# IvanAnishchuk/eth-consensus-specs

Hardware: AMD Instinct MI355X
Metric: BLS sig verifications/sec (FastAggregateVerify, 1/8 GPU) + % int VALU peak (higher is better)
Workload: dtype u32 (381-bit Montgomery Fp, radix-2^29 digits); 1 GPU; C2 sync-committee FastAggregateVerify: 10000 aggregates x 512 pubkeys per GPU; config=c2, global_batch=10000, registry=1048576, parallelism=dp1 (sharded, RCCL all-gather of 576-B Fp12 partials)

## Files before the change

__graft_entry__.py:

```python
import os
import subprocess
import sys

ROOT = os.path.dirname(os.path.abspath(__file__))
PKG = os.path.join(ROOT, "eth-consensus-specs_amd")


def _paths():
    for p in (ROOT, PKG):
        if p not in sys.path:
            sys.path.insert(0, p)


def build() -> None:
    subprocess.check_call(["make", "-C", PKG, "-j8"], timeout=3000)
    subprocess.check_call(["make", "-j2", "-C", os.path.join(ROOT, "tests", "hostcheck")], timeout=3000)
    subprocess.check_call(["make", "-C", os.path.join(ROOT, "tests", "hostcheck_endo")], timeout=3000)
    subprocess.check_call(["make", "-C", os.path.join(ROOT, "tests", "hostcheck_mlines")], timeout=3000)
    subprocess.check_call(["make", "-C", os.path.join(ROOT, "tests", "hostcheck_segsum")], timeout=3000)
    subprocess.check_call(["make", "-C", os.path.join(ROOT, "tests", "hostcheck_g2segsum")], timeout=3000)
    subprocess.check_call(["make", "-C", os.path.join(ROOT, "tests", "hostcheck_g1dot")], timeout=3000)
    subprocess.check_call(["make", "-C", os.path.join(ROOT, "tests", "hostcheck_bits")], timeout=3000)
    subprocess.check_call(["make", "-C", os.path.join(ROOT, "oracle")], timeout=3000)
    subprocess.check_call(["make", "-j3", "-C", os.path.join(ROOT, "tests", "sanitize")], timeout=3000)
    _paths()
    import bls_mi355x
    from bls_mi355x import _native
    _native.load_library()


def smoke() -> None:
    _paths()
    import hashlib

    from bls_mi355x import batch
    from bls_mi355x import bls as shim
    from oracle import bls_oracle as O

    n = 64
    sks = b"".join((i + 1).to_bytes(32, "big") for i in range(n))
    pks = batch.sk_to_pk_batch(sks)
    assert pks[:48] == O.SkToPk(1)
    batch.Registry().load(pks)
    committees = [list(range(0, 16)), list(range(16, 48)), list(range(48, 64))]
    msgs = [hashlib.sha256(bytes([j])).digest() for j in range(3)]
    agg = [sum(k + 1 for k in c) % O.R for c in committees]
    sigs = bytearray(batch.sign_batch(b"".join(a.to_bytes(32, "big") for a in agg), b"".join(msgs)))
    sigs[96:192] = sigs[192:288]
    idx = [k for c in committees for k in c]
    offs = batch.offsets_from_lengths([len(c) for c in committees])
    out = batch.fast_aggregate_verify_batch(idx, offs, b"".join(msgs), bytes(sigs))
    expect = [O.FastAggregateVerify([pks[48 * k: 48 * k + 48] for k in c], m, bytes(sigs[96 * j: 96 * j + 96]))
              for j, (c, m) in enumerate(zip(committees, msgs))]
    assert list(out) == expect == [True, False, True], (list(out), expect)
    pk, m = O.SkToPk(7), b"\x12" * 32
    assert shim.Verify(pk, m, O.Sign(7, m)) is True
    print("smoke ok:", list(out))


if __name__ == "__main__":
    build()
    if len(sys.argv) > 1 and sys.argv[1] == "smoke":
        smoke()
```

eth-consensus-specs_amd/csrc/bls_fq.h:

```cpp
#pragma once
#include "bls_fp.h"
#include "bls_fq_constants.h"

#ifdef BLS_FQ_CHECK
#include <assert.h>
#endif

namespace bls {

constexpr uint32_t Q29_MASK = 0x1fffffffu;

#ifdef BLS_FQ_CHECK
inline double fq_check_top(const Fq& a) {
  double v = 0;
  for (int i = 0; i < 14; ++i) v += (double)a.d[i] * __builtin_ldexp(1.0, 29 * i - 377);
  return v;
}
inline void fq_check_mul(const Fq& x, const Fq& y) {
  assert(fq_check_top(x) * fq_check_top(y) < 13.0 * __builtin_ldexp(1.0, 29));
}
#define FQ_CHECK_MUL(x, y) fq_check_mul(x, y)
inline void fq_check_dot2(const Fq& x, const Fq& y, const Fq& u, const Fq& v) {
  assert(fq_check_top(x) * fq_check_top(y) + fq_check_top(u) * fq_check_top(v) < 13.0 * __builtin_ldexp(1.0, 29));
}
#define FQ_CHECK_DOT2(x, y, u, v) fq_check_dot2(x, y, u, v)
#define FQ_CHECK_COL(acc128) assert((acc128) < ((unsigned __int128)1 << 64))
#define FQ_CHECK_SUB(b, K)                                        \
  do {                                                            \
    for (int i_ = 0; i_ < 14; ++i_) assert((b).d[i_] <= (K)[i_]); \
  } while (0)
#else
#define FQ_CHECK_MUL(x, y) ((void)0)
#define FQ_CHECK_DOT2(x, y, u, v) ((void)0)
#define FQ_CHECK_COL(acc128) ((void)0)
#define FQ_CHECK_SUB(b, K) ((void)0)
#endif

BLS_HD Fq fq_zero() {
  Fq r;
#pragma unroll
  for (int i = 0; i < 14; i++) r.d[i] = 0;
  return r;
}

BLS_HD Fq fq_select(bool c, const Fq& a, const Fq& b) {
  Fq r;
#pragma unroll
  for (int i = 0; i < 14; i++) r.d[i] = c ? a.d[i] : b.d[i];
  return r;
}

BLS_HD Fq fq_add(const Fq& a, const Fq& b) {
  Fq r;
#pragma unroll
  for (int i = 0; i < 14; i++) r.d[i] = a.d[i] + b.d[i];
  return r;
}

BLS_HD Fq fq_sub(const Fq& a, const Fq& b) {
  FQ_CHECK_SUB(b, Q29_K1);
  Fq r;
#pragma unroll
  for (int i = 0; i < 14; i++) r.d[i] = a.d[i] + (Q29_K1[i] - b.d[i]);
  return r;
}

BLS_HD Fq fq_sub2(const Fq& a, const Fq& b) {
  FQ_CHECK_SUB(b, Q29_K2);
  Fq r;
#pragma unroll
  for (int i = 0; i < 14; i++) r.d[i] = a.d[i] + (Q29_K2[i] - b.d[i]);
  return r;
}

BLS_HD Fq fq_norm(const Fq& a) {
  Fq r;
  r.d[0] = a.d[0] & Q29_MASK;
#pragma unroll
  for (int i = 1; i < 13; i++) r.d[i] = (a.d[i] & Q29_MASK) + (a.d[i - 1] >> 29);
  r.d[13] = a.d[13] + (a.d[12] >> 29);
  return r;
}

BLS_HD Fq fq_mul_small(const Fq& a, uint32_t k) {
  uint64_t t[14];
#pragma unroll
  for (int i = 0; i < 14; i++) t[i] = (uint64_t)a.d[i] * k;
  Fq r;
  r.d[0] = (uint32_t)t[0] & Q29_MASK;
#pragma unroll
  for (int i = 1; i < 13; i++) r.d[i] = ((uint32_t)t[i] & Q29_MASK) + (uint32_t)(t[i - 1] >> 29);
  r.d[13] = (uint32_t)t[13] + (uint32_t)(t[12] >> 29);
  return r;
}

BLS_HD Fq fq_mul(const Fq& x, const Fq& y) {
  FQ_CHECK_MUL(x, y);
  uint32_t m[14];
  Fq r;
  uint64_t acc = 0;
#pragma unroll
  for (int k = 0; k < 27; k++) {
#ifdef BLS_FQ_CHECK
    unsigned __int128 chk = acc;
#endif
#pragma unroll
    for (int i = 0; i < 14; i++) {
      const int j = k - i;
      if (j >= 0 && j < 14) {
        acc += (uint64_t)x.d[i] * y.d[j];
#ifdef BLS_FQ_CHECK
        chk += (unsigned __int128)x.d[i] * y.d[j];
#endif
      }
    }
#pragma unroll
    for (int i = 0; i < 14; i++) {
      const int j = k - i;
      if (j >= 1 && j < 14 && i < k) {
        acc += (uint64_t)m[i] * P29[j];
#ifdef BLS_FQ_CHECK
        chk += (unsigned __int128)m[i] * P29[j];
#endif
      }
    }
    if (k < 14) {
      m[k] = ((uint32_t)acc * P29_NINV) & Q29_MASK;
      acc += (uint64_t)m[k] * P29[0];
#ifdef BLS_FQ_CHECK
      chk += (unsigned __int128)m[k] * P29[0];
#endif
    } else {
      r.d[k - 14] = (uint32_t)acc & Q29_MASK;
    }
    FQ_CHECK_COL(chk);
    acc >>= 29;
  }
  r.d[13] = (uint32_t)acc;
  return r;
}

BLS_HD Fq fq_mul_dot2(const Fq& x, const Fq& y, const Fq& u, const Fq& v) {
  FQ_CHECK_DOT2(x, y, u, v);
  uint32_t m[14];
  Fq r;
  uint64_t acc = 0;
#pragma unroll
  for (int k = 0; k < 27; k++) {
#ifdef BLS_FQ_CHECK
    unsigned __int128 chk = acc;
#endif
#pragma unroll
    for (int i = 0; i < 14; i++) {
      const int j = k - i;
      if (j >= 0 && j < 14) {
        acc += (uint64_t)x.d[i] * y.d[j];
        acc += (uint64_t)u.d[i] * v.d[j];
#ifdef BLS_FQ_CHECK
        chk += (unsigned __int128)x.d[i] * y.d[j] + (unsigned __int128)u.d[i] * v.d[j];
#endif
      }
    }
#pragma unroll
    for (int i = 0; i < 14; i++) {
      const int j = k - i;
      if (j >= 1 && j < 14 && i < k) {
        acc += (uint64_t)m[i] * P29[j];
#ifdef BLS_FQ_CHECK
        chk += (unsigned __int128)m[i] * P29[j];
#endif
      }
    }
    if (k < 14) {
      m[k] = ((uint32_t)acc * P29_NINV) & Q29_MASK;
      acc += (uint64_t)m[k] * P29[0];
#ifdef BLS_FQ_CHECK
      chk += (unsigned __int128)m[k] * P29[0];
#endif
    } else {
      r.d[k - 14] = (uint32_t)acc & Q29_MASK;
    }
    FQ_CHECK_COL(chk);
    acc >>= 29;
  }
  r.d[13] = (uint32_t)acc;
  return r;
}

BLS_HD Fq fq_sqr(const Fq& x) {
  FQ_CHECK_MUL(x, x);
  uint32_t m[14];
  Fq r;
  uint64_t acc = 0;
#pragma unroll
  for (int k = 0; k < 27; k++) {
    uint64_t od = 0;
#pragma unroll
    for (int i = 0; i < 14; i++) {
      const int j = k - i;
      if (j > i && j < 14) od += (uint64_t)x.d[i] * x.d[j];
    }
#ifdef BLS_FQ_CHECK
    unsigned __int128 chk = (unsigned __int128)acc + 2 * (unsigned __int128)od;
#endif
    acc += od << 1;
    if ((k & 1) == 0 && (k >> 1) < 14) {
      acc += (uint64_t)x.d[k >> 1] * x.d[k >> 1];
#ifdef BLS_FQ_CHECK
      chk += (unsigned __int128)x.d[k >> 1] * x.d[k >> 1];
#endif
    }
#pragma unroll
    for (int i = 0; i < 14; i++) {
      const int j = k - i;
      if (j >= 1 && j < 14 && i < k) {
        acc += (uint64_t)m[i] * P29[j];
#ifdef BLS_FQ_CHECK
        chk += (unsigned __int128)m[i] * P29[j];
#endif
      }
    }
    if (k < 14) {
      m[k] = ((uint32_t)acc * P29_NINV) & Q29_MASK;
      acc += (uint64_t)m[k] * P29[0];
#ifdef BLS_FQ_CHECK
      chk += (unsigned __int128)m[k] * P29[0];
#endif
    } else {
      r.d[k - 14] = (uint32_t)acc & Q29_MASK;
    }
    FQ_CHECK_COL(chk);
    acc >>= 29;
  }
  r.d[13] = (uint32_t)acc;
  return r;
}

BLS_HD Fq fq_unpack(const Fp& a) {
  Fq r;
  fp_unpack29(r.d, a);
  return r;
}
BLS_HD Fp fq_pack(const Fq& a) {
  const Fq t = fq_mul(a, fq_unpack(FP_ONE));
  return fp_reduce_once(fp_pack29(t.d));
}
BLS_HD Fp fq_pack_n(const Fq& a) { return fp_reduce_once(fp_pack29(a.d)); }

BLS_HD Fq fq_pow_w3(const Fq& a, const uint32_t* e, int nbits) {
  const Fq a2 = fq_sqr(a);
  const Fq t1 = a;
  const Fq t3 = fq_mul(t1, a2);
  const Fq t5 = fq_mul(t3, a2);
  const Fq t7 = fq_mul(t5, a2);
  Fq r = t1;
  bool started = false;
  int i = nbits - 1;
  while (i >= 0) {
    if (!((e[i >> 5] >> (i & 31)) & 1u)) {
      r = fq_sqr(r);
      --i;
      continue;
    }
    int j = i - 2 < 0 ? 0 : i - 2;
    while (!((e[j >> 5] >> (j & 31)) & 1u)) ++j;
    uint32_t w = 0;
    for (int k = i; k >= j; --k) w = (w << 1) | ((e[k >> 5] >> (k & 31)) & 1u);
    const Fq m = fq_select(w == 1u, t1, fq_select(w == 3u, t3, fq_select(w == 5u, t5, t7)));
// ... 14 lines not shown
```

eth-consensus-specs_amd/csrc/bls_fqb.h:

```cpp
#pragma once
#include "bls_fq.h"

namespace bls {

namespace fqb_detail {
constexpr uint64_t MASK = Q29_MASK;
constexpr uint64_t R_OVER_P = 41291124;
constexpr uint64_t top(uint64_t V) { return (V * 13002090ull + 999999ull) / 1000000ull; }

constexpr bool columns_fit(uint64_t dx, uint64_t tx, uint64_t dy, uint64_t ty) {
  for (int k = 0; k < 27; ++k) {
    unsigned __int128 s = (unsigned __int128)1 << 35;
    for (int i = 0; i < 14; ++i) {
      const int j = k - i;
      if (j < 0 || j > 13) continue;
      s += (unsigned __int128)(i == 13 ? tx : dx) * (j == 13 ? ty : dy);
      s += (unsigned __int128)MASK * P29[j];
    }
    if (s >= ((unsigned __int128)1 << 64)) return false;
  }
  return true;
}

constexpr bool columns_fit2(uint64_t dx, uint64_t tx, uint64_t dy, uint64_t ty, uint64_t du, uint64_t tu, uint64_t dv,
                            uint64_t tv) {
  for (int k = 0; k < 27; ++k) {
    unsigned __int128 s = (unsigned __int128)1 << 35;
    for (int i = 0; i < 14; ++i) {
      const int j = k - i;
      if (j < 0 || j > 13) continue;
      s += (unsigned __int128)(i == 13 ? tx : dx) * (j == 13 ? ty : dy);
      s += (unsigned __int128)(i == 13 ? tu : du) * (j == 13 ? tv : dv);
      s += (unsigned __int128)MASK * P29[j];
    }
    if (s >= ((unsigned __int128)1 << 64)) return false;
  }
  return true;
}

struct KConst {
  uint32_t d[14];
  uint64_t c, max;
  bool ok;
};
constexpr KConst make_k(uint64_t c, uint64_t lo) {
  KConst k{};
  uint64_t w[14] = {};
  uint64_t carry = 0;
  for (int i = 0; i < 14; ++i) {
    const uint64_t t = (uint64_t)P29[i] * c + carry;
    w[i] = i < 13 ? (t & MASK) : t;
    carry = i < 13 ? (t >> 29) : 0;
  }
  uint64_t e_prev = 0, mx = 0;
  k.ok = true;
  for (int i = 0; i < 13; ++i) {
    uint64_t e = 0;
    while (w[i] + (e << 29) < lo + e_prev) ++e;
    const uint64_t v = w[i] + (e << 29) - e_prev;
    if (v > 0xffffffffull) k.ok = false;
    k.d[i] = (uint32_t)v;
    mx = v > mx ? v : mx;
    e_prev = e;
  }
  if (w[13] < e_prev || w[13] - e_prev > 0xffffffffull) k.ok = false;
  k.d[13] = (uint32_t)(w[13] - e_prev);
  k.max = mx > k.d[13] ? mx : k.d[13];
  k.c = c;
  return k;
}
constexpr KConst k_for(uint64_t V, uint64_t D) {
  for (uint64_t c = 1; c < (1ull << 24); ++c) {
    const KConst k = make_k(c, D);
    if (k.ok && k.d[13] >= top(V)) return k;
  }
  return KConst{};
}
template <uint64_t V, uint64_t D>
struct KFor {
  static constexpr KConst k = k_for(V, D);
  static_assert(k.ok, "no subtraction constant covers this subtrahend");
};
}

template <uint64_t V, uint64_t D>
struct FqB {
  static_assert(V >= 1 && V <= (1ull << 24), "value bound out of range");
  static_assert(D <= 0xffffffffull, "digit bound exceeds 32 bits");
  static_assert(fqb_detail::top(V) <= 0xffffffffull, "top digit exceeds 32 bits");
  static constexpr uint64_t val = V, dig = D;
  Fq x;
};
using FqN = FqB<2, fqb_detail::MASK>;
using FqC = FqB<1, fqb_detail::MASK>;

template <uint64_t V, uint64_t D>
BLS_HD FqB<V, D> fqb(const Fq& x) {
  return FqB<V, D>{x};
}
BLS_HD FqC fqb_canon(const Fp& a) { return FqC{fq_unpack(a)}; }

template <uint64_t V1, uint64_t D1, uint64_t V2, uint64_t D2>
BLS_HD FqB<V1 + V2, D1 + D2> operator+(const FqB<V1, D1>& a, const FqB<V2, D2>& b) {
  return {fq_add(a.x, b.x)};
}

template <uint64_t V1, uint64_t D1, uint64_t V2, uint64_t D2>
BLS_HD FqB<V1 + fqb_detail::KFor<V2, D2>::k.c, D1 + fqb_detail::KFor<V2, D2>::k.max> operator-(const FqB<V1, D1>& a,
                                                                                                const FqB<V2, D2>& b) {
  constexpr fqb_detail::KConst K = fqb_detail::KFor<V2, D2>::k;
  Fq r;
#pragma unroll
  for (int i = 0; i < 14; i++) r.d[i] = a.x.d[i] + (K.d[i] - b.x.d[i]);
  return {r};
}

template <uint64_t V, uint64_t D>
BLS_HD FqB<V, fqb_detail::MASK + (D >> 29)> norm(const FqB<V, D>& a) {
  return {fq_norm(a.x)};
}

template <uint64_t K, uint64_t V, uint64_t D>
BLS_HD FqB<K * V, fqb_detail::MASK + ((K * D) >> 29)> small(const FqB<V, D>& a) {
  static_assert(K * D < (1ull << 61), "small multiple overflows");
  return {fq_mul_small(a.x, (uint32_t)K)};
}

template <uint64_t V1, uint64_t D1, uint64_t V2, uint64_t D2>
BLS_HD FqN operator*(const FqB<V1, D1>& a, const FqB<V2, D2>& b) {
  static_assert(V1 * V2 <= fqb_detail::R_OVER_P, "product operand values exceed p R");
  static_assert(fqb_detail::columns_fit(D1, fqb_detail::top(V1), D2, fqb_detail::top(V2)),
                "product column exceeds 64 bits");
  return {fq_mul(a.x, b.x)};
}
template <uint64_t V1, uint64_t D1, uint64_t V2, uint64_t D2, uint64_t V3, uint64_t D3, uint64_t V4, uint64_t D4>
BLS_HD FqN dot2(const FqB<V1, D1>& a, const FqB<V2, D2>& b, const FqB<V3, D3>& c, const FqB<V4, D4>& d) {
  static_assert(V1 * V2 + V3 * V4 <= fqb_detail::R_OVER_P, "dot product operand values exceed p R");
  static_assert(fqb_detail::columns_fit2(D1, fqb_detail::top(V1), D2, fqb_detail::top(V2), D3, fqb_detail::top(V3), D4,
                                         fqb_detail::top(V4)),
                "dot product column exceeds 64 bits");
  return {fq_mul_dot2(a.x, b.x, c.x, d.x)};
}
template <uint64_t V, uint64_t D>
BLS_HD FqB<fqb_detail::KFor<V, D>::k.c, fqb_detail::KFor<V, D>::k.max> neg(const FqB<V, D>& b) {
  constexpr fqb_detail::KConst K = fqb_detail::KFor<V, D>::k;
  Fq r;
#pragma unroll
  for (int i = 0; i < 14; i++) r.d[i] = K.d[i] - b.x.d[i];
  return {r};
}
template <class A, class B, class C, class D>
constexpr bool dot2_fits() {
  return fqb_detail::columns_fit2(A::dig, fqb_detail::top(A::val), B::dig, fqb_detail::top(B::val), C::dig,
                                  fqb_detail::top(C::val), D::dig, fqb_detail::top(D::val));
}

template <uint64_t V, uint64_t D>
BLS_HD FqN sqr(const FqB<V, D>& a) {
  static_assert(V * V <= fqb_detail::R_OVER_P, "square operand value exceeds sqrt(p R)");
  static_assert(fqb_detail::columns_fit(D, fqb_detail::top(V), D, fqb_detail::top(V)), "square column exceeds 64 bits");
  return {fq_sqr(a.x)};
}

template <uint64_t V, uint64_t D, uint64_t V1, uint64_t D1>
BLS_HD FqB<V, D> relax(const FqB<V1, D1>& a) {
  static_assert(V1 <= V && D1 <= D, "value does not fit the declared bound");
  return {a.x};
}
template <uint64_t V1, uint64_t D1, uint64_t V2, uint64_t D2>
BLS_HD FqB<(V1 > V2 ? V1 : V2), (D1 > D2 ? D1 : D2)> sel(bool c, const FqB<V1, D1>& a, const FqB<V2, D2>& b) {
  return {fq_select(c, a.x, b.x)};
}

template <uint64_t V, uint64_t D>
struct Fq2B {
  FqB<V, D> c0, c1;
};
template <uint64_t V, uint64_t D>
BLS_HD Fq2B<V, D> fq2b(const FqB<V, D>& c0, const FqB<V, D>& c1) {
  return {c0, c1};
}
template <uint64_t V, uint64_t D>
BLS_HD Fq2B<V, D> fq2b_zero() {
  return {{fq_zero()}, {fq_zero()}};
}

template <uint64_t V1, uint64_t D1, uint64_t V2, uint64_t D2>
BLS_HD auto operator+(const Fq2B<V1, D1>& a, const Fq2B<V2, D2>& b) {
  return Fq2B<V1 + V2, D1 + D2>{a.c0 + b.c0, a.c1 + b.c1};
}
template <uint64_t V1, uint64_t D1, uint64_t V2, uint64_t D2>
BLS_HD auto operator-(const Fq2B<V1, D1>& a, const Fq2B<V2, D2>& b) {
  using R = decltype(a.c0 - b.c0);
  return Fq2B<R::val, R::dig>{a.c0 - b.c0, a.c1 - b.c1};
}
template <uint64_t V, uint64_t D>
BLS_HD auto norm(const Fq2B<V, D>& a) {
  using R = decltype(norm(a.c0));
  return Fq2B<R::val, R::dig>{norm(a.c0), norm(a.c1)};
}
template <uint64_t K, uint64_t V, uint64_t D>
BLS_HD auto small(const Fq2B<V, D>& a) {
  using R = decltype(small<K>(a.c0));
  return Fq2B<R::val, R::dig>{small<K>(a.c0), small<K>(a.c1)};
}
template <uint64_t V, uint64_t D, uint64_t V1, uint64_t D1>
BLS_HD Fq2B<V, D> relax(const Fq2B<V1, D1>& a) {
  return {relax<V, D>(a.c0), relax<V, D>(a.c1)};
}
template <uint64_t V1, uint64_t D1, uint64_t V2, uint64_t D2>
BLS_HD auto sel(bool c, const Fq2B<V1, D1>& a, const Fq2B<V2, D2>& b) {
  using R = decltype(sel(c, a.c0, b.c0));
  return Fq2B<R::val, R::dig>{sel(c, a.c0, b.c0), sel(c, a.c1, b.c1)};
}
template <uint64_t V, uint64_t D>
BLS_HD auto xi(const Fq2B<V, D>& a) {
  using R0 = decltype(a.c0 - a.c1);
  using R = FqB<(R0::val > 2 * V ? R0::val : 2 * V), (R0::dig > 2 * D ? R0::dig : 2 * D)>;
  return Fq2B<R::val, R::dig>{relax<R::val, R::dig>(a.c0 - a.c1), relax<R::val, R::dig>(a.c0 + a.c1)};
}
template <uint64_t V1, uint64_t D1, uint64_t V2, uint64_t D2>
BLS_HD Fq2B<2, fqb_detail::MASK> operator*(const Fq2B<V1, D1>& a, const Fq2B<V2, D2>& b) {
  const auto nb = neg(b.c1);
  using A = FqB<V1, D1>;
  using B = FqB<V2, D2>;
// ... 66 lines not shown
```

eth-consensus-specs_amd/csrc/bls_miller_pair.hip:

```cpp
#include <type_traits>

#include "bls_fqb.h"
#include "bls_kernels.h"
#include "bls_miller_lines.h"
#include "bls_tower_inline.h"

namespace bls {

namespace {

constexpr uint64_t ML_QF_V = 256, ML_QF_D = 0x20000000ull + 64;

#define SEQ() __builtin_amdgcn_sched_barrier(0)

__device__ __forceinline__ uint32_t dpp_q(uint32_t v) {
  return (uint32_t)__builtin_amdgcn_mov_dpp((int)v, 0xB1, 0xF, 0xF, false);
}
__device__ __forceinline__ uint32_t dpp_h(uint32_t v) {
  return (uint32_t)__builtin_amdgcn_mov_dpp((int)v, 0x4E, 0xF, 0xF, false);
}
template <int CTRL>
__device__ __forceinline__ uint32_t dpp_b(uint32_t v) {
  return (uint32_t)__builtin_amdgcn_mov_dpp((int)v, CTRL, 0xF, 0xF, false);
}
constexpr int BQ0 = 0xA0, BQ1 = 0xF5, BH0 = 0x44, BH1 = 0xEE;

}

namespace {

template <uint64_t V, uint64_t D>
__device__ __forceinline__ FqB<V, D> dq(const FqB<V, D>& a) {
  Fq r;
#pragma unroll
  for (int i = 0; i < 14; i++) r.d[i] = dpp_q(a.x.d[i]);
  return {r};
}
template <uint64_t V, uint64_t D>
__device__ __forceinline__ FqB<V, D> dh(const FqB<V, D>& a) {
  Fq r;
#pragma unroll
  for (int i = 0; i < 14; i++) r.d[i] = dpp_h(a.x.d[i]);
  return {r};
}
template <uint64_t V, uint64_t D>
__device__ __forceinline__ Fq2B<V, D> dq2(const Fq2B<V, D>& a) {
  return {dq(a.c0), dq(a.c1)};
}
template <uint64_t V, uint64_t D>
__device__ __forceinline__ Fq2B<V, D> dh2(const Fq2B<V, D>& a) {
  return {dh(a.c0), dh(a.c1)};
}
template <uint64_t V, uint64_t D>
__device__ __forceinline__ Fq6B<V, D> dh6(const Fq6B<V, D>& a) {
  return {dh2(a.c0), dh2(a.c1), dh2(a.c2)};
}
template <int CTRL, uint64_t V, uint64_t D>
__device__ __forceinline__ FqB<V, D> bc(const FqB<V, D>& a) {
  Fq r;
#pragma unroll
  for (int i = 0; i < 14; i++) r.d[i] = dpp_b<CTRL>(a.x.d[i]);
  return {r};
}
template <int CTRL, uint64_t V, uint64_t D>
__device__ __forceinline__ Fq2B<V, D> bc2(const Fq2B<V, D>& a) {
  return {bc<CTRL>(a.c0), bc<CTRL>(a.c1)};
}
template <int CTRL, uint64_t V, uint64_t D>
__device__ __forceinline__ Fq6B<V, D> bc6(const Fq6B<V, D>& a) {
  return {bc2<CTRL>(a.c0), bc2<CTRL>(a.c1), bc2<CTRL>(a.c2)};
}

template <uint64_t VX, uint64_t DX, uint64_t VY, uint64_t DY>
__device__ __forceinline__ auto qq6mul(const Fq6B<VX, DX>& X, const Fq6B<VY, DY>& Y, bool q) {
  const auto p0 = sel(q, norm(X.c1 + X.c2), X.c0) * sel(q, norm(Y.c1 + Y.c2), Y.c0);
  SEQ();
  const auto p1 = sel(q, norm(X.c0 + X.c1), X.c1) * sel(q, norm(Y.c0 + Y.c1), Y.c1);
  SEQ();
  const auto p2 = sel(q, norm(X.c0 + X.c2), X.c2) * sel(q, norm(Y.c0 + Y.c2), Y.c2);
  SEQ();
  const auto t0 = bc2<BQ0>(p0), t1 = bc2<BQ0>(p1), t2 = bc2<BQ0>(p2);
  const auto u0 = bc2<BQ1>(p0), u1 = bc2<BQ1>(p1), u2 = bc2<BQ1>(p2);
  const auto c0 = norm(xi(norm(u0 - (t1 + t2))) + t0);
  const auto c1 = norm((u1 - (t0 + t1)) + xi(t2));
  const auto c2 = norm((u2 - (t0 + t2)) + t1);
  return fq6b(c0, c1, c2);
}

template <uint64_t V, uint64_t D>
__device__ __forceinline__ auto qq_sqr(const Fq6B<V, D>& own, bool h, bool q) {
  const auto o = dh6(own);
  const auto X = norm(sel(h, o, own + o));
  const auto Y = norm(sel(h, own, own + f6v(o)));
  const auto P = qq6mul(X, Y, q);
  const auto t = bc6<BH1>(P);
  return norm(sel(h, P + P, (P - t) - f6v(t)));
}

template <uint64_t V, uint64_t D, uint64_t VL, uint64_t DL, uint64_t VM, uint64_t DM>
__device__ __forceinline__ auto qq_line(const Fq6B<V, D>& own, bool h, bool q, const Fq2B<VL, DL>& l0,
                                        const Fq2B<VM, DM>& l2, const Fq2B<VM, DM>& l3) {
  const auto p1 = sel(q, norm(own.c0 + own.c1), own.c0) * sel(q, norm(l0 + l2), l0);
  SEQ();
  const auto p2 = sel(q, dh2(own.c2), own.c1) * sel(q, l3, l2);
  SEQ();
  const auto p3 = sel(q, dh2(own.c0), own.c2) * sel(q, l3, l2);
  SEQ();
  const auto p4 = sel(q, dh2(own.c1), own.c2) * sel(q, l3, l0);
  SEQ();
  const auto t0 = bc2<BQ0>(p1), t1 = bc2<BQ0>(p2), u0 = bc2<BQ0>(p3), u2 = bc2<BQ0>(p4);
  const auto u1 = bc2<BQ1>(p1), v0 = bc2<BQ1>(p2), v1 = bc2<BQ1>(p3), v2 = bc2<BQ1>(p4);
  const auto m01 = fq6b(t0 + xi(u0), (u1 - (t0 + t1)), t1 + u2);
  const auto m1 = fq6b(xi(v0), v1, v2);
  return norm(norm(m01) + sel(h, m1, f6v(m1)));
}

struct LineIn {
  Fq2B<ML_LV, ML_LD> l0;
  FqB<ML_LV, ML_LD> c;
};
__device__ __forceinline__ LineIn ld_line(const uint32_t* Li, size_t n, bool h, bool q) {
  LineIn r;
#pragma unroll
  for (int j = 0; j < 14; ++j) {
    r.l0.c0.x.d[j] = Li[(size_t)j * n];
    r.l0.c1.x.d[j] = Li[(size_t)(14 + j) * n];
  }
  const uint32_t* Lc = Li + (size_t)((h ? 56 : 28) + (q ? 14 : 0)) * n;
#pragma unroll
  for (int j = 0; j < 14; ++j) r.c.x.d[j] = Lc[(size_t)j * n];
  return r;
}

struct LineS {
  Fq2B<ML_LV, ML_LD> l0;
  Fq2B<2, fqb_detail::MASK> l2, l3;
};
__device__ __forceinline__ LineS ld_line_s(const uint32_t* Li, size_t n) {
  LineS r;
#pragma unroll
  for (int j = 0; j < 14; ++j) {
    r.l0.c0.x.d[j] = Li[(size_t)j * n];
    r.l0.c1.x.d[j] = Li[(size_t)(14 + j) * n];
    r.l2.c0.x.d[j] = Li[(size_t)(28 + j) * n];
    r.l2.c1.x.d[j] = Li[(size_t)(42 + j) * n];
    r.l3.c0.x.d[j] = Li[(size_t)(56 + j) * n];
    r.l3.c1.x.d[j] = Li[(size_t)(70 + j) * n];
  }
  return r;
}

template <uint64_t VP, uint64_t DP>
__device__ __forceinline__ void qq_line_p(const LineIn& in, const FqB<VP, DP>& pc, bool q, Fq2B<2, fqb_detail::MASK>& l2,
                                          Fq2B<2, fqb_detail::MASK>& l3) {
  const FqN mine = in.c * pc;
  const Fq2B<2, fqb_detail::MASK> m{bc<BQ0>(mine), bc<BQ1>(mine)};
  l2 = bc2<BH0>(m);
  l3 = bc2<BH1>(m);
}

}

template <int G>
__global__ void __launch_bounds__(64) k_miller_acc4q(const G1A* P, const G2A* Q, const int* ok, size_t n,
                                                     const uint32_t* L, size_t ld, Fp12* out) {
  const size_t t = (size_t)blockIdx.x * 64 + threadIdx.x;
  const size_t grp = t >> 2;
  const bool h = (t & 2) != 0, q = (t & 1) != 0;
  const size_t ngrp = (n + G - 1) / G;
  if (grp >= ngrp) return;
  bool live[G];
  size_t pi[G];
  bool any = false;
#pragma unroll
  for (int g = 0; g < G; ++g) {
    const size_t p = grp * G + g;
    pi[g] = p < n ? p : n - 1;
    live[g] = p < n && (!ok || ok[p]) && !P[p].inf && !Q[p].inf;
    any = any || live[g];
  }
  if (!any) {
    if (!q) {
      Fp6* o = h ? &out[grp].c1 : &out[grp].c0;
      *o = h ? Fp6{fp2_zero(), fp2_zero(), fp2_zero()} : Fp6{fp2_one(), fp2_zero(), fp2_zero()};
    }
    return;
  }
  constexpr uint64_t VF = ML_QF_V, DF = ML_QF_D;
  using F = Fq6B<VF, DF>;
  const size_t step = (size_t)ML_WORDS * ld;
  const uint32_t* Lb[G];
#pragma unroll
  for (int g = 0; g < G; ++g) Lb[g] = L + pi[g];
  const FqC one = fqb_canon(FP_ONE), zero{fq_zero()};
  const Fq2B<1, fqb_detail::MASK> z2{zero, zero};
  F f = relax<VF, DF>(Fq6B<1, fqb_detail::MASK>{{sel(h, zero, one), zero}, z2, z2});
  using PcT = decltype(sel(h, zero, zero - zero));
// ... 99 lines not shown
  const auto y0 = dq2(x0);
  const auto y1 = dq2(x1);
  const auto y2 = dq2(x2);
  const auto X = fq6b(sel(q, y0, x0), sel(q, y1, x1), sel(q, y2, x2));
  const auto Y = fq6b(sel(q, x0, y0), sel(q, x1, y1), sel(q, x2, y2));
  const auto K = qq6mul(X, Y, q);
  const auto e0 = bc2<BL0>(e);
  const auto e1 = bc2<BL1>(e);
  const auto e2 = bc2<BL2>(e);
  const auto DD = fq6b(xi(norm(e2 - (e0 + e1))), xi(e1), e0);
  const auto K0 = bc6<BH0>(K);
  return norm(sel(h, norm(K - norm(K0 + DD)), norm(K0 + f6v(DD))));
}

template <uint64_t V, uint64_t D>
__device__ __forceinline__ void park6(uint32_t* lds, const Fq6B<V, D>& f, int lane) {
  const uint32_t* w = reinterpret_cast<const uint32_t*>(&f);
#pragma unroll
  for (int i = 0; i < 84; ++i) lds[i * 64 + lane] = w[i];
}
template <uint64_t V, uint64_t D>
__device__ __forceinline__ Fq6B<V, D> unpark6(const uint32_t* lds, int lane) {
  Fq6B<V, D> f;
  uint32_t* w = reinterpret_cast<uint32_t*>(&f);
  __asm__ volatile("" ::: "memory");
#pragma unroll
  for (int i = 0; i < 84; ++i) w[i] = lds[i * 64 + lane];
  return f;
}

template <uint64_t V, uint64_t D, uint64_t VM, uint64_t DM>
__device__ __forceinline__ auto ll_fm(const uint32_t* fpark, const Fq6B<VM, DM>& M, bool h, bool q, int lane) {
  auto f = unpark6<V, D>(fpark, lane);
  const auto Z = qq6mul(f, M, q);
  SEQ();
  const auto X = norm(f + dh6(f));
  const auto xa = sel(h, sel(q, norm(X.c1 + X.c2), X.c2), sel(q, X.c1, X.c0));
  const auto xb = sel(q, norm(X.c0 + X.c2), norm(X.c0 + X.c1));
  const auto Y = norm(M + dh6(M));
  const auto ya = sel(h, sel(q, norm(Y.c1 + Y.c2), Y.c2), sel(q, Y.c1, Y.c0));
  const auto yb = sel(q, norm(Y.c0 + Y.c2), norm(Y.c0 + Y.c1));
  const auto pa = xa * ya;
  SEQ();
  const auto pb = xb * yb;
  SEQ();
  const auto r0 = bc2<BL0>(pa), r1 = bc2<BL1>(pa), r2 = bc2<BL2>(pa), r3 = bc2<BL3>(pa);
  const auto s0 = bc2<BL0>(pb), s1 = bc2<BL1>(pb);
  const auto S = fq6b(norm(xi(norm(r3 - (r1 + r2))) + r0), norm((s0 - (r0 + r1)) + xi(r2)),
                      norm((s1 - (r0 + r2)) + r1));
  const auto Zo = dh6(Z);
  return norm(sel(h, S - norm(Z + Zo), Z + f6v(Zo)));
}

}

__global__ void __launch_bounds__(64) k_miller_acc4l(const G1A* P, const G2A* Q, const int* ok, size_t n,
                                                     const uint32_t* L, size_t ld, Fp12* out) {
  constexpr int G = 4;
  const size_t t = (size_t)blockIdx.x * 64 + threadIdx.x;
  const size_t grp = t >> 2;
  const bool h = (t & 2) != 0, q = (t & 1) != 0;
  const size_t ngrp = (n + G - 1) / G;
  if (grp >= ngrp) return;
  bool any = false, live[2];
  size_t pi[2];
#pragma unroll
  for (int g = 0; g < G; ++g) {
    const size_t p = grp * G + g;
    const size_t pc = p < n ? p : n - 1;
    const bool lv = p < n && (!ok || ok[p]) && !P[p].inf && !Q[p].inf;
    any = any || lv;
    if ((g >> 1) == (int)q) {
      live[g & 1] = lv;
      pi[g & 1] = pc;
    }
  }
  if (!any) {
    if (!q) {
      Fp6* o = h ? &out[grp].c1 : &out[grp].c0;
      *o = h ? Fp6{fp2_zero(), fp2_zero(), fp2_zero()} : Fp6{fp2_one(), fp2_zero(), fp2_zero()};
    }
    return;
  }
  constexpr uint64_t VF = ML_QF_V, DF = ML_QF_D;
  using F = Fq6B<VF, DF>;
  const size_t step = (size_t)ML_WORDS * ld;
  const uint32_t* La = L + pi[0];
  const uint32_t* Lb = L + pi[1];
  const FqC one = fqb_canon(FP_ONE), zero{fq_zero()};
  const Fq2B<1, fqb_detail::MASK> z2{zero, zero};
  F f = relax<VF, DF>(Fq6B<1, fqb_detail::MASK>{{sel(h, zero, one), zero}, z2, z2});
  using PcT = decltype(sel(h, zero, zero - zero));
  __shared__ uint32_t pcs[2][14][64];
  __shared__ uint32_t fpark[84 * 64];
  const int lane = (int)threadIdx.x;
#pragma unroll
  for (int s = 0; s < 2; ++s) {
    const FqC pv = fqb_canon(h ? P[pi[s]].y : P[pi[s]].x);
    const PcT pcg = sel(h, pv, zero - pv);
#pragma unroll
    for (int w = 0; w < 14; ++w) pcs[s][w][lane] = pcg.x.d[w];
  }
#pragma unroll 1
  for (int b = 62; b >= 0; --b) {
    if (b != 62) f = relax<VF, DF>(qq_sqr(f, h, q));
    const int nl = ((X_ABS >> b) & 1ull) ? 2 : 1;
#pragma unroll 1
    for (int s = 0; s < nl; ++s) {
      __asm__ volatile("" : "+v"(La), "+v"(Lb));
      const LineRaw ra = ld_line_raw(La, ld, h);
      const LineRaw rb = ld_line_raw(Lb, ld, h);
      park6(fpark, f, lane);
      SEQ();
      PcT pa, pb;
#pragma unroll
      for (int w = 0; w < 14; ++w) pa.x.d[w] = pcs[0][w][lane];
      const LineF A = line_f(ra, h, pa, live[0]);
      SEQ();
#pragma unroll
      for (int w = 0; w < 14; ++w) pb.x.d[w] = pcs[1][w][lane];
      const LineF B = line_f(rb, h, pb, live[1]);
      SEQ();
      const auto M = ll_m(A, B, h, q);
      SEQ();
      f = relax<VF, DF>(ll_fm<VF, DF>(fpark, M, h, q, lane));
      SEQ();
      La += step;
      Lb += step;
    }
  }
  if (!q) {
    Fp6 r{fq2b_pack(f.c0), fq2b_pack(f.c1), fq2b_pack(f.c2)};
    if (h)
      out[grp].c1 = Fp6{fp2_neg(r.c0), fp2_neg(r.c1), fp2_neg(r.c2)};
    else
      out[grp].c0 = r;
  }
}

namespace {

__device__ __forceinline__ uint32_t dpp_m(uint32_t v) {
  return (uint32_t)__builtin_amdgcn_mov_dpp((int)v, 0x141, 0xF, 0xF, false);
}
template <uint64_t V, uint64_t D>
__device__ __forceinline__ FqB<V, D> dm(const FqB<V, D>& a) {
  Fq r;
#pragma unroll
  for (int i = 0; i < 14; i++) r.d[i] = dpp_m(a.x.d[i]);
  return {r};
}
template <uint64_t V, uint64_t D>
__device__ __forceinline__ Fq2B<V, D> dm2(const Fq2B<V, D>& a) {
  return {dm(a.c0), dm(a.c1)};
}
template <uint64_t V, uint64_t D>
__device__ __forceinline__ Fq6B<V, D> dm6(const Fq6B<V, D>& a) {
  return {dm2(a.c0), dm2(a.c1), dm2(a.c2)};
}

template <uint64_t VX, uint64_t DX, uint64_t VY, uint64_t DY>
__device__ __forceinline__ auto q4_6mul(const Fq6B<VX, DX>& X, const Fq6B<VY, DY>& Y, bool j1, bool j0) {
  const auto p1 = sel(j1, sel(j0, norm(X.c1 + X.c2), X.c2), sel(j0, X.c1, X.c0)) *
                  sel(j1, sel(j0, norm(Y.c1 + Y.c2), Y.c2), sel(j0, Y.c1, Y.c0));
  SEQ();
  const auto p2 = sel(j0, norm(X.c0 + X.c2), norm(X.c0 + X.c1)) * sel(j0, norm(Y.c0 + Y.c2), norm(Y.c0 + Y.c1));
  SEQ();
  const auto r0 = bc2<BL0>(p1), r1 = bc2<BL1>(p1), r2 = bc2<BL2>(p1), r3 = bc2<BL3>(p1);
  const auto s0 = bc2<BL0>(p2), s1 = bc2<BL1>(p2);
  const auto c0 = norm(xi(norm(r3 - (r1 + r2))) + r0);
  const auto c1 = norm((s0 - (r0 + r1)) + xi(r2));
  const auto c2 = norm((s1 - (r0 + r2)) + r1);
  return fq6b(c0, c1, c2);
}

template <uint64_t V, uint64_t D>
__device__ __forceinline__ auto q8_sqr(const Fq6B<V, D>& own, bool h, bool j1, bool j0) {
  const auto o = dm6(own);
  const auto X = norm(sel(h, o, own + o));
  const auto Y = norm(sel(h, own, own + f6v(o)));
  const auto P = q4_6mul(X, Y, j1, j0);
  const auto t = dm6(P);
  return norm(sel(h, P + P, (P - t) - f6v(t)));
}

template <uint64_t V, uint64_t D, uint64_t VL, uint64_t DL, uint64_t VM, uint64_t DM>
__device__ __forceinline__ auto q8_line(const Fq6B<V, D>& own, bool h, bool j1, bool j0, const Fq2B<VL, DL>& l0,
                                        const Fq2B<VM, DM>& l2, const Fq2B<VM, DM>& l3) {
  const auto pa = sel(j1, own.c2, sel(j0, own.c1, own.c0)) * sel(j1, sel(j0, l0, l2), sel(j0, l2, l0));
  SEQ();
  const auto o = dm6(own);
  const auto pb = sel(j1, sel(j0, o.c1, o.c0), sel(j0, o.c2, norm(own.c0 + own.c1))) *
                  sel(j1, l3, sel(j0, l3, norm(l0 + l2)));
  SEQ();
  const auto t0 = bc2<BL0>(pa), t1 = bc2<BL1>(pa), u0 = bc2<BL2>(pa), u2 = bc2<BL3>(pa);
  const auto u1 = bc2<BL0>(pb), v0 = bc2<BL1>(pb), v1 = bc2<BL2>(pb), v2 = bc2<BL3>(pb);
  const auto m01 = fq6b(t0 + xi(u0), (u1 - (t0 + t1)), t1 + u2);
  const auto m1 = fq6b(xi(v0), v1, v2);
  return norm(norm(m01) + sel(h, m1, f6v(m1)));
}

}

__global__ void __launch_bounds__(64) k_miller_acc8(const G1A* P, const G2A* Q, const int* ok, size_t n,
                                                    const uint32_t* L, size_t ld, Fp12* out) {
  const size_t t = (size_t)blockIdx.x * 64 + threadIdx.x;
  const size_t pi = t >> 3;
  const bool h = (t & 4) != 0, j1 = (t & 2) != 0, j0 = (t & 1) != 0;
  if (pi >= n) return;
  const bool live = (!ok || ok[pi]) && !P[pi].inf && !Q[pi].inf;
  if (!live) {
    if (!j1 && !j0) {
      Fp6* o = h ? &out[pi].c1 : &out[pi].c0;
      *o = h ? Fp6{fp2_zero(), fp2_zero(), fp2_zero()} : Fp6{fp2_one(), fp2_zero(), fp2_zero()};
    }
    return;
  }
  constexpr uint64_t VF = ML_QF_V, DF = ML_QF_D;
  using F = Fq6B<VF, DF>;
  const size_t step = (size_t)ML_WORDS * ld;
  const uint32_t* Lp = L + pi;
  const FqC one = fqb_canon(FP_ONE), zero{fq_zero()};
  const Fq2B<1, fqb_detail::MASK> z2{zero, zero};
  F f = relax<VF, DF>(Fq6B<1, fqb_detail::MASK>{{sel(h, zero, one), zero}, z2, z2});
  const FqC pv = fqb_canon(h ? P[pi].y : P[pi].x);
  const auto pc = sel(h, pv, zero - pv);
#pragma unroll 1
  for (int b = 62; b >= 0; --b) {
    if (b != 62) f = relax<VF, DF>(q8_sqr(f, h, j1, j0));
    const int nl = ((X_ABS >> b) & 1ull) ? 2 : 1;
#pragma unroll 1
    for (int s = 0; s < nl; ++s) {
      const LineIn cur = ld_line(Lp, ld, h, j0);
      const FqN mine = cur.c * pc;
      const Fq2B<2, fqb_detail::MASK> m{bc<BL0>(mine), bc<BL1>(mine)};
      const auto mo = dm2(m);
      const auto l2 = sel(h, mo, m), l3 = sel(h, m, mo);
      f = relax<VF, DF>(q8_line(f, h, j1, j0, cur.l0, l2, l3));
      Lp += step;
    }
  }
  if (!j1 && !j0) {
    Fp6 r{fq2b_pack(f.c0), fq2b_pack(f.c1), fq2b_pack(f.c2)};
    if (h)
      out[pi].c1 = Fp6{fp2_neg(r.c0), fp2_neg(r.c1), fp2_neg(r.c2)};
    else
      out[pi].c0 = r;
  }
}

template <int G>
constexpr int MF_PAIRS = G == 2 ? 64 : 32;
template <int G>
constexpr int MF_ACC = 4 * MF_PAIRS<G> / G / 64;

template <int G>
__global__ void __launch_bounds__(64 * (1 + MF_ACC<G>)) k_miller_fused(const G1A* P, const G2A* Q, const int* ok,
                                                                       size_t n, Fp12* out) {
  constexpr int PW = MF_PAIRS<G>;
  __shared__ uint32_t rec[2][ML_WORDS * PW];
  __shared__ uint32_t qlds[56 * 64];
  const int wave = (int)(threadIdx.x >> 6), lane = (int)(threadIdx.x & 63);
  const size_t pair0 = (size_t)blockIdx.x * PW;
  if (wave == 0) {
    constexpr int LPP = 64 / PW;
    const int pl = lane / LPP;
    const size_t i = pair0 + pl < n ? pair0 + pl : n - 1;
    G2A q = Q[i];
    if (q.inf) q = g2_generator();
    using LT = typename std::conditional<LPP == 1, mlines::Line1<true>, mlines::Line2<true>>::type;
    LT T;
    if constexpr (LPP == 1)
      T.init(q, qlds, lane);
    else
      T.init(q, (lane & 1) != 0, qlds, lane);
    T.pf.init(P[i]);
    uint32_t* const r0 = &rec[0][pl];
    uint32_t* const r1 = &rec[1][pl];
    T.dbl(r0, PW);
    __syncthreads();
    int b = 62;
    bool added = false;
#pragma unroll 1
    for (int k = 1; k <= MILLER_NLINES; ++k) {
      if (k < MILLER_NLINES) {
        uint32_t* dst = (k & 1) ? r1 : r0;
        if (!added && ((X_ABS >> b) & 1ull)) {
          T.add(dst, PW, qlds, lane);
          added = true;
        } else {
          --b;
          added = false;
          T.dbl(dst, PW);
        }
      }
      __syncthreads();
    }
    return;
  }
  const int at = (wave - 1) * 64 + lane;
  const int grp = at >> 2;
// ... 94 lines not shown
```

Baseline: 2.772 million FAV/s.

## Replace per-lane Fp6 products in Miller loop with fused six-term Montgomery dot products

```diff
diff --git a/__graft_entry__.py b/__graft_entry__.py
--- a/__graft_entry__.py
+++ b/__graft_entry__.py
@@ -21,6 +21,7 @@
     subprocess.check_call(["make", "-C", os.path.join(ROOT, "tests", "hostcheck_g2segsum")], timeout=3000)
     subprocess.check_call(["make", "-C", os.path.join(ROOT, "tests", "hostcheck_g1dot")], timeout=3000)
     subprocess.check_call(["make", "-C", os.path.join(ROOT, "tests", "hostcheck_bits")], timeout=3000)
+    subprocess.check_call(["make", "-C", os.path.join(ROOT, "tests", "hostcheck_accdot")], timeout=3000)
     subprocess.check_call(["make", "-C", os.path.join(ROOT, "oracle")], timeout=3000)
     subprocess.check_call(["make", "-j3", "-C", os.path.join(ROOT, "tests", "sanitize")], timeout=3000)
     _paths()
diff --git a/eth-consensus-specs_amd/csrc/bls_acc_dot.h b/eth-consensus-specs_amd/csrc/bls_acc_dot.h
--- /dev/null
+++ b/eth-consensus-specs_amd/csrc/bls_acc_dot.h
@@ -0,0 +1,103 @@
+#pragma once
+#include "bls_fqb.h"
+
+namespace bls {
+namespace accdot {
+
+#if defined(__HIP_DEVICE_COMPILE__)
+#define ACC_SEQ() __builtin_amdgcn_sched_barrier(0)
+#else
+#define ACC_SEQ() ((void)0)
+#endif
+
+using N2 = Fq2B<2, fqb_detail::MASK>;
+using N6 = Fq6B<2, fqb_detail::MASK>;
+
+constexpr uint64_t ACC_YD = 0x20000000ull + 64;
+template <uint64_t V, uint64_t D>
+BLS_HD auto fit(const FqB<V, D>& a) {
+  if constexpr (D > ACC_YD)
+    return norm(a);
+  else
+    return a;
+}
+
+template <class A, class B>
+struct YP {
+  A a;
+  B b;
+};
+template <class A, class B>
+BLS_HD YP<A, B> yp(const A& a, const B& b) {
+  return {a, b};
+}
+template <uint64_t V, uint64_t D>
+BLS_HD auto prep(const Fq2B<V, D>& y, bool q) {
+  return yp(fit(sel(q, y.c1, y.c0)), fit(sel(q, y.c0, neg(y.c1))));
+}
+template <uint64_t V, uint64_t D>
+BLS_HD auto prep_xi(const Fq2B<V, D>& y, bool q) {
+  const auto d = y.c0 + neg(y.c1);
+  const auto s = y.c0 + y.c1;
+  return yp(fit(sel(q, s, d)), fit(sel(q, d, neg(s))));
+}
+template <class A1, class B1, class A2, class B2>
+BLS_HD auto sel(bool c, const YP<A1, B1>& x, const YP<A2, B2>& y) {
+  return yp(sel(c, x.a, y.a), sel(c, x.b, y.b));
+}
+
+template <uint64_t V0, uint64_t D0, class P0, uint64_t V1, uint64_t D1, class P1, uint64_t V2, uint64_t D2, class P2>
+BLS_HD FqN dot3(const Fq2B<V0, D0>& u0, const P0& p0, const Fq2B<V1, D1>& u1, const P1& p1, const Fq2B<V2, D2>& u2,
+                const P2& p2) {
+  return dot6(u0.c0, p0.a, u1.c0, p1.a, u2.c0, p2.a, u0.c1, p0.b, u1.c1, p1.b, u2.c1, p2.b);
+}
+
+template <int I, uint64_t V, uint64_t D>
+BLS_HD const Fq2B<V, D>& coef(const Fq6B<V, D>& a) {
+  if constexpr (I == 0)
+    return a.c0;
+  else if constexpr (I == 1)
+    return a.c1;
+  else
+    return a.c2;
+}
+
+template <class Ex, uint64_t V, uint64_t D, uint64_t VL, uint64_t DL, uint64_t VM, uint64_t DM>
+BLS_HD void line_lane(const Fq6B<V, D>& own, bool h, bool q, const Fq2B<VL, DL>& l0, const Fq2B<VM, DM>& l2,
+                      const Fq2B<VM, DM>& l3, const Ex& ex, FqN (&r)[3]) {
+  const auto p0 = prep(l0, q);
+  const auto x3 = prep_xi(l3, q);
+  r[0] = dot3(own.c0, p0, own.c2, prep_xi(l2, q), ex.template other<1, 2>(own, h), x3);
+  ACC_SEQ();
+  const auto p2 = prep(l2, q);
+  const auto p3 = prep(l3, q);
+  r[1] = dot3(own.c0, p2, own.c1, p0, ex.template other<2, 0>(own, h), sel(h, p3, x3));
+  ACC_SEQ();
+  r[2] = dot3(own.c1, p2, own.c2, p0, ex.template other<0, 1>(own, h), p3);
+  ACC_SEQ();
+}
+
+template <class Ex, uint64_t V, uint64_t D>
+BLS_HD void sqr_lane(const Fq6B<V, D>& own, bool h, bool q, const Ex& ex, FqN (&r)[3]) {
+  const auto o = ex.half(own);
+  const auto X = norm(sel(h, o, own + o));
+  const auto Y = norm(sel(h, own, own + f6v(o)));
+  const auto p0 = prep(Y.c0, q);
+  const auto x2 = prep_xi(Y.c2, q);
+  r[0] = dot3(X.c0, p0, X.c1, x2, X.c2, prep_xi(Y.c1, q));
+  ACC_SEQ();
+  const auto p1 = prep(Y.c1, q);
+  r[1] = dot3(X.c0, p1, X.c1, p0, X.c2, x2);
+  ACC_SEQ();
+  r[2] = dot3(X.c0, prep(Y.c2, q), X.c1, p1, X.c2, p0);
+  ACC_SEQ();
+}
+BLS_HD auto sqr_fin(const N6& P, const N6& t, bool h) { return norm(sel(h, P + P, (P - t) - f6v(t))); }
+
+}
+
+using AccSqrOut = decltype(accdot::sqr_fin(accdot::N6{}, accdot::N6{}, false).c0.c0);
+constexpr uint64_t ML_QF_V = AccSqrOut::val, ML_QF_D = AccSqrOut::dig;
+static_assert(ML_QF_V == 11 && ML_QF_D == 0x20000000ull + 5, "the bound DESIGN 4.3 and tests/test_accdot_cpu.py state");
+
+}
diff --git a/eth-consensus-specs_amd/csrc/bls_fq.h b/eth-consensus-specs_amd/csrc/bls_fq.h
--- a/eth-consensus-specs_amd/csrc/bls_fq.h
+++ b/eth-consensus-specs_amd/csrc/bls_fq.h
@@ -24,6 +24,7 @@
   assert(fq_check_top(x) * fq_check_top(y) + fq_check_top(u) * fq_check_top(v) < 13.0 * __builtin_ldexp(1.0, 29));
 }
 #define FQ_CHECK_DOT2(x, y, u, v) fq_check_dot2(x, y, u, v)
+#define FQ_CHECK_DOT6(o) fq_check_dot6(o)
 #define FQ_CHECK_COL(acc128) assert((acc128) < ((unsigned __int128)1 << 64))
 #define FQ_CHECK_SUB(b, K)                                        \
   do {                                                            \
@@ -32,6 +33,7 @@
 #else
 #define FQ_CHECK_MUL(x, y) ((void)0)
 #define FQ_CHECK_DOT2(x, y, u, v) ((void)0)
+#define FQ_CHECK_DOT6(o) ((void)0)
 #define FQ_CHECK_COL(acc128) ((void)0)
 #define FQ_CHECK_SUB(b, K) ((void)0)
 #endif
@@ -184,6 +186,80 @@
     acc >>= 29;
   }
   r.d[13] = (uint32_t)acc;
+  return r;
+}
+
+struct FqDot6 {
+  const Fq &x0, &y0, &x1, &y1, &x2, &y2, &x3, &y3, &x4, &y4, &x5, &y5;
+};
+#ifdef BLS_FQ_CHECK
+inline void fq_check_dot6(const FqDot6& o) {
+  assert(fq_check_top(o.x0) * fq_check_top(o.y0) + fq_check_top(o.x1) * fq_check_top(o.y1) +
+             fq_check_top(o.x2) * fq_check_top(o.y2) + fq_check_top(o.x3) * fq_check_top(o.y3) +
+             fq_check_top(o.x4) * fq_check_top(o.y4) + fq_check_top(o.x5) * fq_check_top(o.y5) <
+         13.00208 * __builtin_ldexp(1.0, 29));
+}
+#endif
+template <int K>
+BLS_HD void fq_dot6_cols(const FqDot6& o, uint32_t (&m)[14], Fq& r, uint64_t& A, uint64_t& B) {
+  if constexpr (K < 27) {
+    constexpr int LO = K > 13 ? K - 13 : 0, HI = K < 13 ? K : 13, HR = K - 1 < 13 ? K - 1 : 13;
+#ifdef BLS_FQ_CHECK
+    unsigned __int128 ca = A, cb = B;
+#endif
+#pragma unroll
+    for (int i = LO; i <= HI; i++) {
+      const int j = K - i;
+      A += (uint64_t)o.x0.d[i] * o.y0.d[j];
+      A += (uint64_t)o.x1.d[i] * o.y1.d[j];
+      A += (uint64_t)o.x2.d[i] * o.y2.d[j];
+      B += (uint64_t)o.x3.d[i] * o.y3.d[j];
+      B += (uint64_t)o.x4.d[i] * o.y4.d[j];
+      B += (uint64_t)o.x5.d[i] * o.y5.d[j];
+#ifdef BLS_FQ_CHECK
+      ca += (unsigned __int128)o.x0.d[i] * o.y0.d[j] + (unsigned __int128)o.x1.d[i] * o.y1.d[j] +
+            (unsigned __int128)o.x2.d[i] * o.y2.d[j];
+      cb += (unsigned __int128)o.x3.d[i] * o.y3.d[j] + (unsigned __int128)o.x4.d[i] * o.y4.d[j] +
+            (unsigned __int128)o.x5.d[i] * o.y5.d[j];
+#endif
+    }
+#pragma unroll
+    for (int i = LO; i <= HR; i++) {
+      A += (uint64_t)m[i] * P29[K - i];
+#ifdef BLS_FQ_CHECK
+      ca += (unsigned __int128)m[i] * P29[K - i];
+#endif
+    }
+    const uint32_t bl = (uint32_t)B & Q29_MASK;
+    A += bl;
+#ifdef BLS_FQ_CHECK
+    ca += bl;
+#endif
+    if constexpr (K < 14) {
+      m[K] = ((uint32_t)A * P29_NINV) & Q29_MASK;
+      A += (uint64_t)m[K] * P29[0];
+#ifdef BLS_FQ_CHECK
+      ca += (unsigned __int128)m[K] * P29[0];
+#endif
+    } else {
+      r.d[K - 14] = (uint32_t)A & Q29_MASK;
+    }
+    FQ_CHECK_COL(ca);
+    FQ_CHECK_COL(cb);
+    A >>= 29;
+    B >>= 29;
+    fq_dot6_cols<K + 1>(o, m, r, A, B);
+  }
+}
+BLS_HD Fq fq_mul_dot6(const Fq& x0, const Fq& y0, const Fq& x1, const Fq& y1, const Fq& x2, const Fq& y2, const Fq& x3,
+                      const Fq& y3, const Fq& x4, const Fq& y4, const Fq& x5, const Fq& y5) {
+  const FqDot6 o{x0, y0, x1, y1, x2, y2, x3, y3, x4, y4, x5, y5};
+  FQ_CHECK_DOT6(o);
+  uint32_t m[14];
+  Fq r;
+  uint64_t A = 0, B = 0;
+  fq_dot6_cols<0>(o, m, r, A, B);
+  r.d[13] = (uint32_t)A + (uint32_t)B;
   return r;
 }
 
diff --git a/eth-consensus-specs_amd/csrc/bls_fqb.h b/eth-consensus-specs_amd/csrc/bls_fqb.h
--- a/eth-consensus-specs_amd/csrc/bls_fqb.h
+++ b/eth-consensus-specs_amd/csrc/bls_fqb.h
@@ -38,6 +38,24 @@
   return true;
 }
 
+struct Dot6Bounds {
+  uint64_t dx[6], tx[6], dy[6], ty[6];
+};
+constexpr bool columns_fit6(const Dot6Bounds& b) {
+  for (int k = 0; k < 27; ++k) {
+    unsigned __int128 sa = (unsigned __int128)1 << 36, sb = (unsigned __int128)1 << 35;
+    for (int i = 0; i < 14; ++i) {
+      const int j = k - i;
+      if (j < 0 || j > 13) continue;
+      for (int t = 0; t < 6; ++t)
+        (t < 3 ? sa : sb) += (unsigned __int128)(i == 13 ? b.tx[t] : b.dx[t]) * (j == 13 ? b.ty[t] : b.dy[t]);
+      sa += (unsigned __int128)MASK * P29[j];
+    }
+    if (sa >= ((unsigned __int128)1 << 64) || sb >= ((unsigned __int128)1 << 64)) return false;
+  }
+  return true;
+}
+
 struct KConst {
   uint32_t d[14];
   uint64_t c, max;
@@ -141,6 +159,27 @@
                 "dot product column exceeds 64 bits");
   return {fq_mul_dot2(a.x, b.x, c.x, d.x)};
 }
+template <class X0, class Y0, class X1, class Y1, class X2, class Y2, class X3, class Y3, class X4, class Y4, class X5,
+          class Y5>
+constexpr bool dot6_fits() {
+  using fqb_detail::top;
+  return fqb_detail::columns_fit6(
+      {{X0::dig, X1::dig, X2::dig, X3::dig, X4::dig, X5::dig},
+       {top(X0::val), top(X1::val), top(X2::val), top(X3::val), top(X4::val), top(X5::val)},
+       {Y0::dig, Y1::dig, Y2::dig, Y3::dig, Y4::dig, Y5::dig},
+       {top(Y0::val), top(Y1::val), top(Y2::val), top(Y3::val), top(Y4::val), top(Y5::val)}});
+}
+template <class X0, class Y0, class X1, class Y1, class X2, class Y2, class X3, class Y3, class X4, class Y4, class X5,
+          class Y5>
+BLS_HD FqN dot6(const X0& x0, const Y0& y0, const X1& x1, const Y1& y1, const X2& x2, const Y2& y2, const X3& x3,
+                const Y3& y3, const X4& x4, const Y4& y4, const X5& x5, const Y5& y5) {
+  static_assert(X0::val * Y0::val + X1::val * Y1::val + X2::val * Y2::val + X3::val * Y3::val + X4::val * Y4::val +
+                        X5::val * Y5::val <=
+                    fqb_detail::R_OVER_P,
+                "dot product operand values exceed p R");
+  static_assert(dot6_fits<X0, Y0, X1, Y1, X2, Y2, X3, Y3, X4, Y4, X5, Y5>(), "dot product column exceeds 64 bits");
+  return {fq_mul_dot6(x0.x, y0.x, x1.x, y1.x, x2.x, y2.x, x3.x, y3.x, x4.x, y4.x, x5.x, y5.x)};
+}
 template <uint64_t V, uint64_t D>
 BLS_HD FqB<fqb_detail::KFor<V, D>::k.c, fqb_detail::KFor<V, D>::k.max> neg(const FqB<V, D>& b) {
   constexpr fqb_detail::KConst K = fqb_detail::KFor<V, D>::k;
diff --git a/eth-consensus-specs_amd/csrc/bls_miller_pair.hip b/eth-consensus-specs_amd/csrc/bls_miller_pair.hip
--- a/eth-consensus-specs_amd/csrc/bls_miller_pair.hip
+++ b/eth-consensus-specs_amd/csrc/bls_miller_pair.hip
@@ -1,5 +1,6 @@
 #include <type_traits>
 
+#include "bls_acc_dot.h"
 #include "bls_fqb.h"
 #include "bls_kernels.h"
 #include "bls_miller_lines.h"
@@ -9,7 +10,7 @@
 
 namespace {
 
-constexpr uint64_t ML_QF_V = 256, ML_QF_D = 0x20000000ull + 64;
+constexpr uint64_t ML_QK_V = 256, ML_QK_D = 0x20000000ull + 64;
 
 #define SEQ() __builtin_amdgcn_sched_barrier(0)
 
@@ -87,32 +88,34 @@
   return fq6b(c0, c1, c2);
 }
 
+struct DppEx {
+  template <int A, int B, uint64_t V, uint64_t D>
+  __device__ __forceinline__ Fq2B<V, D> other(const Fq6B<V, D>& own, bool h) const {
+    return dh2(sel(h, accdot::coef<A>(own), accdot::coef<B>(own)));
+  }
+  template <uint64_t V, uint64_t D>
+  __device__ __forceinline__ Fq6B<V, D> half(const Fq6B<V, D>& own) const {
+    return dh6(own);
+  }
+};
+__device__ __forceinline__ accdot::N6 join_q(const FqN (&r)[3]) {
+  return {{bc<BQ0>(r[0]), bc<BQ1>(r[0])}, {bc<BQ0>(r[1]), bc<BQ1>(r[1])}, {bc<BQ0>(r[2]), bc<BQ1>(r[2])}};
+}
+
 template <uint64_t V, uint64_t D>
 __device__ __forceinline__ auto qq_sqr(const Fq6B<V, D>& own, bool h, bool q) {
-  const auto o = dh6(own);
-  const auto X = norm(sel(h, o, own + o));
-  const auto Y = norm(sel(h, own, own + f6v(o)));
-  const auto P = qq6mul(X, Y, q);
-  const auto t = bc6<BH1>(P);
-  return norm(sel(h, P + P, (P - t) - f6v(t)));
+  FqN r[3];
+  accdot::sqr_lane(own, h, q, DppEx{}, r);
+  const accdot::N6 P = join_q(r);
+  return accdot::sqr_fin(P, bc6<BH1>(P), h);
 }
 
 template <uint64_t V, uint64_t D, uint64_t VL, uint64_t DL, uint64_t VM, uint64_t DM>
-__device__ __forceinline__ auto qq_line(const Fq6B<V, D>& own, bool h, bool q, const Fq2B<VL, DL>& l0,
-                                        const Fq2B<VM, DM>& l2, const Fq2B<VM, DM>& l3) {
-  const auto p1 = sel(q, norm(own.c0 + own.c1), own.c0) * sel(q, norm(l0 + l2), l0);
-  SEQ();
-  const auto p2 = sel(q, dh2(own.c2), own.c1) * sel(q, l3, l2);
-  SEQ();
-  const auto p3 = sel(q, dh2(own.c0), own.c2) * sel(q, l3, l2);
-  SEQ();
-  const auto p4 = sel(q, dh2(own.c1), own.c2) * sel(q, l3, l0);
-  SEQ();
-  const auto t0 = bc2<BQ0>(p1), t1 = bc2<BQ0>(p2), u0 = bc2<BQ0>(p3), u2 = bc2<BQ0>(p4);
-  const auto u1 = bc2<BQ1>(p1), v0 = bc2<BQ1>(p2), v1 = bc2<BQ1>(p3), v2 = bc2<BQ1>(p4);
-  const auto m01 = fq6b(t0 + xi(u0), (u1 - (t0 + t1)), t1 + u2);
-  const auto m1 = fq6b(xi(v0), v1, v2);
-  return norm(norm(m01) + sel(h, m1, f6v(m1)));
+__device__ __forceinline__ accdot::N6 qq_line(const Fq6B<V, D>& own, bool h, bool q, const Fq2B<VL, DL>& l0,
+                                              const Fq2B<VM, DM>& l2, const Fq2B<VM, DM>& l3) {
+  FqN r[3];
+  accdot::line_lane(own, h, q, l0, l2, l3, DppEx{}, r);
+  return join_q(r);
 }
 
 struct LineIn {
@@ -378,7 +381,7 @@
     }
     return;
   }
-  constexpr uint64_t VF = ML_QF_V, DF = ML_QF_D;
+  constexpr uint64_t VF = ML_QK_V, DF = ML_QK_D;
   using F = Fq6B<VF, DF>;
   const size_t step = (size_t)ML_WORDS * ld;
   const uint32_t* La = L + pi[0];
@@ -512,7 +515,7 @@
     }
     return;
   }
-  constexpr uint64_t VF = ML_QF_V, DF = ML_QF_D;
+  constexpr uint64_t VF = ML_QK_V, DF = ML_QK_D;
   using F = Fq6B<VF, DF>;
   const size_t step = (size_t)ML_WORDS * ld;
   const uint32_t* Lp = L + pi;
```

Measured after the change: 2.894 million FAV/s (median of 6 runs). +4.4%, better.
